# HuajianUP/Photo-SLAM

Hardware: AMD Instinct MI355X
Metric: train iters/s (render + L1/SSIM loss + backward + Adam), 2M Gaussians @1080p (higher is better)
Workload: dtype f32; 1 GPU; C3: Replica room0 @1080p shape; gaussians=2000000, width=1920, height=1080, sh_degree=3, parallelism=single GPU, raster_only=False, densify_interval=0, cull_empty_tiles=False, binning=depth-first, sh_adam_fused_into_backward=True, sh_adam_lazy_window=32, scene_index_order=random, geometry_adam_fused_into_backward=True, gaussians_after=2000000

## Files before the change

### photo-slam_amd/csrc/gsr_api.hip

```cpp
#include <atomic>
#include <chrono>
#include <cmath>
#include <vector>
#include "kernels.h"
#include "shrows.h"

#include <stdio.h>
#include <stdlib.h>
#include <string.h>

namespace gsr {

static thread_local int t_last_err = 0;
static thread_local char t_last_what[256] = {0};
void set_last_hip_error(int err, const char* what)
{
	t_last_err = err;
	snprintf(t_last_what, sizeof(t_last_what), "%s: %s", what ? what : "?", hipGetErrorString((hipError_t)err));
}

struct HostSync {
	uint32_t* pinned = nullptr;
	uint32_t* pinned_dev = nullptr;
	hipEvent_t ev = nullptr;
	hipStream_t side = nullptr;
	hipEvent_t fork = nullptr, join = nullptr;
	hipEvent_t notify = nullptr;
	int init_notify()
	{
		if (!notify) GSR_HIP(hipEventCreateWithFlags(&notify, hipEventDisableTiming));
		return GSR_OK;
	}
	int init_side()
	{
		if (!side) {
			int lo = 0, hi = 0;
			GSR_HIP(hipDeviceGetStreamPriorityRange(&lo, &hi));
			GSR_HIP(hipStreamCreateWithPriority(&side, hipStreamNonBlocking, lo));
		}
		if (!fork) GSR_HIP(hipEventCreateWithFlags(&fork, hipEventDisableTiming));
		if (!join) GSR_HIP(hipEventCreateWithFlags(&join, hipEventDisableTiming));
		return GSR_OK;
	}
	int init()
	{
		if (pinned && pinned_dev && ev) return GSR_OK;
		if (!pinned) {
			GSR_HIP(hipHostMalloc((void**)&pinned, 64 * sizeof(uint32_t), hipHostMallocMapped));
		}
		if (!pinned_dev) GSR_HIP(hipHostGetDevicePointer((void**)&pinned_dev, pinned, 0));
		if (!ev) GSR_HIP(hipEventCreateWithFlags(&ev, hipEventDisableTiming));
		return GSR_OK;
	}
	void release()
	{
		if (ev) (void)hipEventDestroy(ev);
		if (fork) (void)hipEventDestroy(fork);
		if (join) (void)hipEventDestroy(join);
		if (notify) (void)hipEventDestroy(notify);
		if (side) (void)hipStreamDestroy(side);
		if (pinned) (void)hipHostFree(pinned);
		*this = HostSync();
	}
};
constexpr int MAX_DEVICES = 16;
struct ThreadState {
	HostSync dev[MAX_DEVICES];
	~ThreadState()
	{
		int cur = 0;
		if (hipGetDevice(&cur) != hipSuccess) return;
		for (int d = 0; d < MAX_DEVICES; d++)
			if (dev[d].pinned || dev[d].ev || dev[d].side) {
				if (hipSetDevice(d) == hipSuccess) dev[d].release();
			}
		(void)hipSetDevice(cur);
	}
};
static thread_local ThreadState t_state;
static gsr_status host_sync(HostSync** out)
{
	int d = 0;
	GSR_HIP(hipGetDevice(&d));
	if (d < 0 || d >= MAX_DEVICES) return GSR_ERR_UNSUPPORTED;
	*out = &t_state.dev[d];
	return GSR_OK;
}
static thread_local int t_last_visible = -1;
static thread_local int t_last_forward_only = -1;
static thread_local const char* t_forward_only_geom = nullptr;
static thread_local const char* t_antialias_geom = nullptr;
static thread_local int t_antialias_bit = 0;
static thread_local double t_sync_wait_us = 0.0;
static thread_local long long t_sync_waits = 0;
static int env_int(const char* name, int unset)
{
	const char* e = getenv(name);
	if (!(e && *e)) return unset;
	fprintf(stderr, "[gsr] environment override %s=%s (wins over the API field / the library's default)\n", name, e);
	return atoi(e);
}
static bool side_stream_enabled(const gsr_sh_adam* o)
{
	static const int env = env_int("GSR_SH_ADAM_SIDE_STREAM", -1);
	return env >= 0 ? env != 0 : !(o && o->no_side_stream);
}
static bool lazy_slice_early(const gsr_sh_adam* o)
{
	static const int env = env_int("GSR_LAZY_SLICE_EARLY", -1);
	return env >= 0 ? env != 0 : !(o && o->lazy_slice_late);
}
static bool cov3D_stored()
{
	static const int env = env_int("GSR_COV3D_STORED", 0);
	return env != 0;
}
static bool emit_seeded()
{
	static const int env = env_int("GSR_EMIT_SEEDS", 1);
	return env != 0;
}
static int xcd_deal_mode(int tiles)
{
	static const int env = env_int("GSR_XCD_CHUNK", -1);
	if (env >= 0) return env;
	int c = 8;
	while (c > 1 && tiles < 8 * 16 * c) c >>= 1;
	return c;
}
static bool blend_bwd_half_tiles(int tiles)
{
	const char* e = getenv("GSR_BWD_HALF_TILES");
	if (e && *e) {
		static bool logged = false;
		if (!logged) fprintf(stderr, "[gsr] environment override GSR_BWD_HALF_TILES=%s\n", e);
		logged = true;
		return atoi(e) != 0;
	}
	return tiles >= 24 * 256;
}
static int depth_sort_wide()
{
	static const int on = env_int("GSR_DEPTH_SORT_9BIT", 1);
	static const int bits = env_int("GSR_DEPTH_SORT_BITS", 3 * RADIX_BITS_WIDE);
	if (!on) return 0;
	return (bits >= 1 && bits <= 27 && (div_up(bits, RADIX_BITS_WIDE) & 1)) ? bits : 3 * RADIX_BITS_WIDE;
}
static thread_local long long t_depth_resorts = 0;
static bool emit_hist()
{
	static const int env = env_int("GSR_EMIT_HIST", 1);
	return env != 0;
}
constexpr int TILE_FIRST_MAX_GAUSSIANS = 256 * 1024;
static bool binning_tile_first(int raw_params, int P, int tiles)
{
	static const int env = env_int("GSR_BINNING", -1);
	if (env >= 0) return env != 0;
	if (raw_params & GSR_BINNING_TILE_FIRST) return true;
	if (raw_params & GSR_BINNING_DEPTH_FIRST) return false;
	(void)tiles;
	return P <= TILE_FIRST_MAX_GAUSSIANS;
}
static int side_blocks(const gsr_sh_adam* o)
{
	static const int env = env_int("GSR_SH_ADAM_SIDE_BLOCKS", -1);
	return env >= 0 ? env : (o && o->side_blocks > 0 ? o->side_blocks : 256);
}

enum { ST_PREPROCESS = 0, ST_DEPTH_SORT, ST_OFFSET_SCAN, ST_EMIT, ST_TILE_SORT, ST_TILE_RANGES, ST_TILE_DEPTH_SORT, ST_BLEND_FWD,
       ST_GRAD_MEMSET, ST_BLEND_BWD, ST_PREPROCESS_BWD, ST_COUNT };
constexpr int ST_FWD_COUNT = ST_BLEND_FWD + 1;
static const char* const k_stage_names[ST_COUNT] = {"preprocess_fwd", "depth_sort", "offset_scan", "emit_instances",
                                                    "tile_sort", "tile_ranges", "tile_depth_sort", "blend_fwd", "grad_memset",
                                                    "blend_bwd", "preprocess_bwd"};
struct Profiler {
	std::atomic<int> on{0};
	hipEvent_t fwd[ST_FWD_COUNT + 1] = {};
	hipEvent_t bwd[4] = {};
	std::atomic<bool> created{false}, fwd_done{false}, bwd_done{false};
	int create()
	{
		if (created) return GSR_OK;
		for (auto& e : fwd) GSR_HIP(hipEventCreate(&e));
		for (auto& e : bwd) GSR_HIP(hipEventCreate(&e));
		created = true;
		return GSR_OK;
	}
};
static Profiler t_prof;
#define PROF_FWD(i) do { if (t_prof.on == 1) GSR_HIP(hipEventRecord(t_prof.fwd[i], stream)); } while (0)
#define PROF_BWD(i) do { if (t_prof.on == 1 || (t_prof.on == 2 && ((i) == 1 || (i) == 2))) GSR_HIP(hipEventRecord(t_prof.bwd[i], stream)); } while (0)

static inline size_t geometry_bytes(int P)
{
	size_t b = 0;
	GeometryState::carve(nullptr, (size_t)P, &b);
	return b;
}
static inline size_t binning_bytes(int R, bool forward_only = false, bool contribution = false)
{
	size_t b = 0;
	BinningState::carve(nullptr, (size_t)R, &b, forward_only, contribution);
	return b;
}
static inline size_t image_bytes(int W, int H, bool forward_only = false)
{
	size_t b = 0;
	const size_t T = (size_t)div_up(W, TILE) * div_up(H, TILE);
	ImageState::carve(nullptr, (size_t)W * H, T, &b, forward_only);
	return b;
}

static int validate_common(int P, int D, int M, int W, int H, const void* shs, const void* colors, const void* scales,
                           const void* rotations, const void* cov3D)
{
	if (P < 0 || W <= 0 || H <= 0) return GSR_ERR_INVALID_ARG;
	if ((shs == nullptr) == (colors == nullptr)) return GSR_ERR_INVALID_ARG;
	const bool sr = scales != nullptr && rotations != nullptr;
	if ((scales != nullptr) != (rotations != nullptr)) return GSR_ERR_INVALID_ARG;
	if (sr == (cov3D != nullptr)) return GSR_ERR_INVALID_ARG;
	if (shs) {
		if (D < 0 || D > 3) return GSR_ERR_UNSUPPORTED;
		if (M < (D + 1) * (D + 1)) return GSR_ERR_INVALID_ARG;
	}
	if (div_up(W, TILE) > 65535 || div_up(H, TILE) > 65535) return GSR_ERR_UNSUPPORTED;
	return GSR_OK;
}

static int make_lazy_adam(const gsr_sh_adam& o, const float* shs, int M, LazyAdam& la)
{
	const gsr_sh_adam_lazy& z = *o.lazy;
	if (!o.param || (shs && o.param != shs) || !o.exp_avg || !o.exp_avg_sq || !z.row_step || o.step < 1 || z.window < 2 ||
	    z.window > GSR_SH_LAZY_WINDOW)
		return GSR_ERR_INVALID_ARG;
	if (M != 16 || ((reinterpret_cast<uintptr_t>(o.param) | reinterpret_cast<uintptr_t>(o.exp_avg) | reinterpret_cast<uintptr_t>(o.exp_avg_sq)) & 15))
		return GSR_ERR_UNSUPPORTED;
	static_assert(GSR_SH_LAZY_WINDOW == LAZY_WINDOW_MAX, "gsr.h and kernels.h agree on the window");
	la.param = o.param; la.exp_avg = o.exp_avg; la.exp_avg_sq = o.exp_avg_sq;
	la.row_step = z.row_step; la.step = o.step; la.window = z.window;
	for (int k = 0; k < LAZY_WINDOW_MAX; k++) {
		AdamScalars s{};
		if (k < z.window && o.step - k >= 1)
			s = adam_scalars(k == 0 ? o.lr : z.lr_past[k - 1], k == 0 ? o.lr_tail : z.lr_tail_past[k - 1], o.beta1, o.beta2, o.eps, o.step - k);
		la.t.step_size[k] = s.step_size; la.t.step_size_tail[k] = s.step_size_tail; la.t.inv_sqrt_bc2[k] = s.inv_sqrt_bc2;
	}
	const AdamScalars c = adam_scalars(o.lr, o.lr_tail, o.beta1, o.beta2, o.eps, o.step);
	la.t.b1 = c.b1; la.t.b2 = c.b2; la.t.omb1 = c.omb1; la.t.omb2 = c.omb2; la.t.eps = c.eps;
	return GSR_OK;
}

}

using namespace gsr;

extern "C" {

size_t gsr_geometry_bytes(int P) { return geometry_bytes(P < 0 ? 0 : P); }
size_t gsr_binning_bytes(int R) { return binning_bytes(R < 0 ? 0 : R); }
size_t gsr_pose_grad_scratch_bytes(int P) { return pose_slab_floats(P) * sizeof(float); }
size_t gsr_geom_reg_scratch_bytes(int P) { return reg_slab_floats(P) * sizeof(float); }
size_t gsr_image_bytes(int W, int H) { return (W <= 0 || H <= 0) ? 0 : image_bytes(W, H); }
size_t gsr_binning_bytes_for(int R, int raw_params)
{
	return binning_bytes(R < 0 ? 0 : R, (raw_params & GSR_FORWARD_ONLY) != 0, (raw_params & GSR_CONTRIBUTION) != 0);
}
size_t gsr_image_bytes_for(int W, int H, int raw_params) { return (W <= 0 || H <= 0) ? 0 : image_bytes(W, H, (raw_params & GSR_FORWARD_ONLY) != 0); }
size_t gsr_knn_scratch_bytes(int P) { return knn_scratch_bytes(P < 0 ? 0 : P); }

const char* gsr_strerror(int status)
{
	switch (status) {
		case GSR_OK: return "ok";
		case GSR_ERR_INVALID_ARG: return "invalid argument";
		case GSR_ERR_ALLOC: return "scratch allocation callback returned NULL";
		case GSR_ERR_HIP: return "HIP runtime error";
		case GSR_ERR_UNSUPPORTED: return "unsupported configuration";
		default: return "unknown status";
	}
}
int gsr_last_hip_error(void) { return t_last_err; }
const char* gsr_last_hip_error_string(void) { return t_last_what; }
const char* gsr_backend(void)
{
#ifdef GSR_EMU
	return "emu-wave64";
#else
	return "hip-gfx950";
#endif
}

int gsr_forward(const gsr_forward_args* a, gsr_alloc_fn geometryBuffer, void* geometry_ctx, gsr_alloc_fn binningBuffer,
                void* binning_ctx, gsr_alloc_fn imageBuffer, void* image_ctx, void* stream_, int* num_rendered)
{
	if (!a || !geometryBuffer || !binningBuffer || !imageBuffer || !num_rendered) return GSR_ERR_INVALID_ARG;
	*num_rendered = 0;
	const bool fwd_only = (a->raw_params & GSR_FORWARD_ONLY) != 0;
	if (fwd_only && a->sh_adam && !a->sh_adam->lazy) return GSR_ERR_INVALID_ARG;
	const bool contribution = (a->raw_params & GSR_CONTRIBUTION) != 0;
	if (contribution != (a->out_weight_sum || a->out_weight_max || a->out_n_touched)) return GSR_ERR_INVALID_ARG;
	if (!contribution && a->pixel_weight) return GSR_ERR_INVALID_ARG;
	t_last_forward_only = fwd_only ? 1 : 0;
	int st = validate_common(a->P, a->D, a->M, a->width, a->height, a->shs, a->colors_precomp, a->scales, a->rotations,
	                         a->cov3D_precomp);
	if (a->P == 0) {
		t_last_visible = 0;
		return GSR_OK;
	}
	if (st != GSR_OK) return st;
	if (!a->background || !a->means3D || !a->opacities || !a->viewmatrix || !a->projmatrix || !a->cam_pos || !a->out_color)
		return GSR_ERR_INVALID_ARG;
	hipStream_t stream = (hipStream_t)stream_;
	const int P = a->P, W = a->width, H = a->height;
	const int grid_x = div_up(W, TILE), grid_y = div_up(H, TILE), tiles = grid_x * grid_y;

	char* geom_chunk = geometryBuffer(geometry_ctx, geometry_bytes(P));
	if (!geom_chunk) return GSR_ERR_ALLOC;
	GeometryState g = GeometryState::carve(geom_chunk, (size_t)P);
	if (fwd_only) t_forward_only_geom = geom_chunk;
	else if (t_forward_only_geom == geom_chunk) t_forward_only_geom = nullptr;
	if (!fwd_only) {
		t_antialias_geom = geom_chunk;
		t_antialias_bit = a->raw_params & GSR_ANTIALIAS;
	}
	char* img_chunk = imageBuffer(image_ctx, image_bytes(W, H, fwd_only));
	if (!img_chunk) return GSR_ERR_ALLOC;
	ImageState im = ImageState::carve(img_chunk, (size_t)W * H, (size_t)tiles, nullptr, fwd_only);

	HostSync* sync_ = nullptr;
	if ((st = host_sync(&sync_)) != GSR_OK) return st;
	HostSync& t_sync = *sync_;
	if ((st = t_sync.init()) != GSR_OK) return st;
	t_prof.fwd_done = false;
	PROF_FWD(0);

	PreprocessParams pp;
	pp.P = P; pp.D = a->D; pp.M = a->M;
	pp.means3D = a->means3D; pp.scales = a->scales; pp.scale_modifier = a->scale_modifier; pp.rotations = a->rotations;
	pp.opacities = a->opacities; pp.shs = a->shs; pp.cov3D_precomp = a->cov3D_precomp; pp.colors_precomp = a->colors_precomp;
	pp.view = a->viewmatrix; pp.proj = a->projmatrix; pp.campos = a->cam_pos;
	pp.W = W; pp.H = H; pp.tan_fovx = a->tan_fovx; pp.tan_fovy = a->tan_fovy;
	pp.focal_y = H / (2.0f * a->tan_fovy);
	pp.focal_x = W / (2.0f * a->tan_fovx);
	pp.grid_x = grid_x; pp.grid_y = grid_y; pp.radii_out = a->radii;
	pp.raw_params = a->raw_params | (cov3D_stored() ? GSR_STORE_COV3D : 0);
	pp.ranges = im.ranges; pp.tiles = tiles;
	pp.lazy = LazyAdam{};
	pp.forward_only = fwd_only ? 1 : 0;
	if (a->sh_adam && a->sh_adam->lazy) {
		if (!a->shs) return GSR_ERR_INVALID_ARG;
		if ((st = make_lazy_adam(*a->sh_adam, a->shs, a->M, pp.lazy)) != GSR_OK) return st;
	}
	if ((st = launch_preprocess_fwd(pp, g, stream)) != GSR_OK) return st;

	PROF_FWD(1);
	RadixHostCount hc;
	hc.pairs = g.wave_counts; hc.n = (int)wave_count_slots((size_t)P); hc.partials = g.count_partials; hc.host_out = t_sync.pinned_dev; hc.ready = t_sync.ev;

	uint32_t* const long_runs = fwd_only ? nullptr : g.long_runs;
	uint32_t* const long_counts = fwd_only ? nullptr : g.long_counts;
	const uint32_t long_capacity = fwd_only ? 0u : g.long_capacity;
	uint32_t *kres = nullptr, *vres = nullptr;
	const int narrow_bits = depth_sort_wide();
	auto plain_depth_sort = [&](const RadixHostCount* ride) {
		return launch_radix_sort(g.depth_key, nullptr, g.sort_keys_a, g.order, g.sort_keys_b, g.sort_vals_b, P, 0, 32, g.sort_scratch, stream,
		                         &kres, &vres, g.visible, ride);
	};
	auto offset_scan = [&]() {
		return launch_scan_rect_tiles(reinterpret_cast<const uint2*>(g.rect), g.order, g.offsets, g.rect_sorted, P, g.scan_scratch, stream,
		                              g.visible, g.sort_keys_b, EMIT_SEED_STRIDE, (uint32_t)P, long_runs, long_counts, long_capacity);
	};
	const bool tile_first = binning_tile_first(a->raw_params, P, tiles);
	if (tile_first) {
		st = launch_compact_visible(g.tiles_touched, reinterpret_cast<const uint2*>(g.rect), g.wave_counts, hc.n, g.count_partials, g.order, g.offsets,
		                            g.rect_sorted, P, t_sync.pinned_dev, t_sync.ev, stream, g.sort_keys_b, EMIT_SEED_STRIDE, (uint32_t)P, long_runs,
		                            long_counts, long_capacity, g.visible);
		if (st != GSR_OK) return st;
		PROF_FWD(2);
	} else {
		if (narrow_bits) {
			st = launch_radix_sort(g.depth_key, nullptr, g.sort_keys_b, g.sort_vals_b, g.sort_keys_a, g.order, P, 0, narrow_bits, g.sort_scratch, stream,
			                       &kres, &vres, g.visible, &hc, false, RADIX_BITS_WIDE, DEPTH_KEY_BIAS);
			if (st == GSR_OK && vres != g.order) st = GSR_ERR_INVALID_ARG;
		} else
			st = plain_depth_sort(&hc);
		if (st != GSR_OK) return st;
		PROF_FWD(2);
		if ((st = offset_scan()) != GSR_OK) return st;
	}
	PROF_FWD(3);

	{
		const auto w0 = std::chrono::steady_clock::now();
		GSR_HIP(hipEventSynchronize(t_sync.ev));
		t_sync_wait_us += std::chrono::duration<double, std::micro>(std::chrono::steady_clock::now() - w0).count();
		t_sync_waits++;
	}
	const unsigned long long R64 = (unsigned long long)t_sync.pinned[0] | ((unsigned long long)t_sync.pinned[1] << 32);
	const unsigned long long V64 = t_sync.pinned[2];
	t_last_visible = (int)V64;
	if (!tile_first && narrow_bits && V64 != 0 && (t_sync.pinned[3] - DEPTH_KEY_BIAS) >> narrow_bits) {
		if (!fwd_only) GSR_HIP(hipMemsetAsync(g.long_counts, 0, (size_t)LONG_LISTS * LONG_COUNT_STRIDE * sizeof(uint32_t), stream));
		if ((st = plain_depth_sort(nullptr)) != GSR_OK) return st;
		if ((st = offset_scan()) != GSR_OK) return st;
		t_depth_resorts++;
	}
	if (R64 > 0x7FFFFFFFull) return GSR_ERR_UNSUPPORTED;
	const int R = (int)R64;
	char* bin_chunk = binningBuffer(binning_ctx, binning_bytes(R, fwd_only, contribution));
	if (!bin_chunk) return GSR_ERR_ALLOC;
	BinningState bs = BinningState::carve(bin_chunk, (size_t)R, nullptr, fwd_only, contribution);

	uint32_t* point_list = bs.vals_a;
	if (R > 0) {
		const int bits = (int)higher_msb((uint32_t)tiles);
		const bool cull = (a->raw_params & GSR_CULL_EMPTY_TILES) != 0 && bits > 0;
		uint32_t* const listed = cull ? g.visible + 16 : nullptr;
		const int digit_bits = tile_sort_digit_bits(tiles, R);
		const bool one_pass = digit_bits == RADIX_BITS_ONE_PASS;
		const int hist_bits = emit_hist() ? radix_first_pass_bits(0, bits, digit_bits) : 0;
		if ((st = launch_emit_instances(tile_first ? (int)V64 : P, R, g, grid_x, bs.keys_a, bs.vals_a, bs.touched, stream, cull ? 1 : 0, emit_seeded(), bs.sort_scratch, hist_bits)) != GSR_OK) return st;
		PROF_FWD(4);
		uint32_t* tkeys = nullptr;
		if ((st = launch_radix_sort(bs.keys_a, bs.vals_a, bs.keys_a, bs.vals_a, bs.keys_b, bs.vals_b, R, 0, bits,
		                            bs.sort_scratch, stream, &tkeys, &point_list, listed, nullptr, hist_bits > 0, digit_bits, 0u,
		                            one_pass ? im.ranges : (uint2*)nullptr)) != GSR_OK)
			return st;
		PROF_FWD(5);
		if (!one_pass && (st = launch_tile_ranges(R, tkeys, im.ranges, stream, listed)) != GSR_OK) return st;
		PROF_FWD(6);
		if (tile_first) {
			const bool in_a = point_list == bs.vals_a;
			if ((st = launch_tile_depth_sort(im.ranges, tiles, g.depth_key, point_list, in_a ? bs.keys_b : bs.keys_a, in_a ? bs.vals_b : bs.vals_a,
			                                 bs.spare_words, stream)) != GSR_OK)
				return st;
		}
	} else {
		PROF_FWD(4);
		PROF_FWD(5);
		PROF_FWD(6);
	}
	PROF_FWD(7);

	BlendFwdParams bp;
	bp.ranges = im.ranges; bp.point_list = point_list; bp.rec = g.rec; bp.bg = a->background;
	bp.final_T = im.final_T; bp.n_contrib = im.n_contrib; bp.out_color = a->out_color;
	bp.contrib = bs.contrib; bp.contrib_stride = (size_t)R;
	bp.W = W; bp.H = H; bp.grid_x = grid_x; bp.tiles = tiles;
	bp.deal = make_tile_deal(tiles, grid_x, xcd_deal_mode(tiles));
	bp.forward_only = fwd_only ? 1 : 0;
	bp.depth = reinterpret_cast<const float*>(g.depth_key);
	bp.out_depth = a->out_depth; bp.out_alpha = a->out_alpha;
	bp.stats = nullptr; bp.stats_slots = (uint32_t)R; bp.pixel_weight = nullptr;
	if (contribution && R > 0) {
		GSR_HIP(hipMemsetAsync(bs.stats, 0, stats_floats((size_t)R) * sizeof(float), stream));
		bp.stats = bs.stats; bp.pixel_weight = a->pixel_weight;
	}
	if ((st = launch_blend_fwd(bp, stream)) != GSR_OK) return st;
	if (contribution) {
		ContributionParams cp;
		cp.P = P; cp.tiles_touched = g.tiles_touched; cp.rec = g.rec; cp.stats = R > 0 ? bs.stats : nullptr; cp.stats_slots = (uint32_t)R;
		cp.out_sum = a->out_weight_sum; cp.out_max = a->out_weight_max; cp.out_cnt = a->out_n_touched;
		cp.accumulate = a->contribution_accumulate ? 1 : 0;
		if ((st = launch_contribution_reduce(cp, stream)) != GSR_OK) return st;
	}
	PROF_FWD(8);
	t_prof.fwd_done = t_prof.on == 1;
	*num_rendered = R;
	return GSR_OK;
}

int gsr_backward(const gsr_backward_args* a, void* stream_)
{
	if (!a) return GSR_ERR_INVALID_ARG;
	int st = validate_common(a->P, a->D, a->M, a->width, a->height, a->shs, a->colors_precomp, a->scales, a->rotations,
	                         a->cov3D_precomp);
	const int pose_ptrs = (a->dL_dviewmatrix != nullptr) + (a->dL_dprojmatrix != nullptr) + (a->dL_dcampos != nullptr) + (a->pose_scratch != nullptr);
	if (pose_ptrs != 0 && pose_ptrs != 4) return GSR_ERR_INVALID_ARG;
	const bool pose = pose_ptrs == 4;
	if (pose && (reinterpret_cast<uintptr_t>(a->pose_scratch) & 3)) return GSR_ERR_INVALID_ARG;
	bool reg = false;
	if (const gsr_geom_reg* gr = a->geom_reg) {
		const float ws[3] = {gr->w_opacity, gr->w_scale, gr->w_isotropic};
		for (const float w : ws)
			if (!std::isfinite(w) || w < 0.f) return GSR_ERR_INVALID_ARG;
		if (gr->loss && (!gr->scratch || (reinterpret_cast<uintptr_t>(gr->scratch) & 3))) return GSR_ERR_INVALID_ARG;
		if (a->cov3D_precomp && (gr->w_scale != 0.f || gr->w_isotropic != 0.f)) return GSR_ERR_INVALID_ARG;
		reg = gr->w_opacity != 0.f || gr->w_scale != 0.f || gr->w_isotropic != 0.f || gr->loss != nullptr;
		if (reg && (a->dL_dcolor_view || a->packed_view || pose)) return GSR_ERR_UNSUPPORTED;
	}
	if (a->P == 0) {
		if (reg && a->geom_reg->loss) return launch_reg_zero(a->geom_reg->loss, (hipStream_t)stream_);
		return pose ? launch_pose_zero(a->dL_dviewmatrix, a->dL_dprojmatrix, a->dL_dcampos, (hipStream_t)stream_) : GSR_OK;
	}
	if (st != GSR_OK) return st;
	if (!a->background || !a->means3D || !a->viewmatrix || !a->projmatrix || !a->campos || !a->geom_buffer ||
	    !a->image_buffer || !a->dL_dpix || !a->dL_dcolor || !a->dL_dmean3D || a->R < 0)
		return GSR_ERR_INVALID_ARG;
	if (pose && (a->dL_dcolor_view || a->packed_view)) return GSR_ERR_UNSUPPORTED;
	if (!a->dL_dopacity && !a->geom_adam) return GSR_ERR_INVALID_ARG;
	if (a->shs && !a->dL_dsh && !a->dL_dcolor_view && !a->sh_adam) return GSR_ERR_INVALID_ARG;
	if ((a->stat_grad_accum != nullptr) != (a->stat_denom != nullptr) || (a->stat_denom != nullptr) != (a->stat_max_radii != nullptr))
		return GSR_ERR_INVALID_ARG;
	if (a->sh_adam && (!a->shs || (a->dL_dcolor_view && !a->sh_adam->lazy) || !a->sh_adam->exp_avg || !a->sh_adam->exp_avg_sq ||
	                   a->sh_adam->step < 1))
		return GSR_ERR_INVALID_ARG;
	if (a->dL_dcolor_view && !a->shs) return GSR_ERR_INVALID_ARG;
	if (a->scales && (!a->dL_dscale || !a->dL_drot) && !a->geom_adam) return GSR_ERR_INVALID_ARG;
	if (a->R > 0 && !a->binning_buffer) return GSR_ERR_INVALID_ARG;
	if (t_forward_only_geom != nullptr && a->geom_buffer == t_forward_only_geom) return GSR_ERR_INVALID_ARG;
	if (t_antialias_geom != nullptr && a->geom_buffer == t_antialias_geom && (a->raw_params & GSR_ANTIALIAS) != t_antialias_bit)
		return GSR_ERR_INVALID_ARG;
	if (a->color_view_ready_stream && a->dL_dcolor_view && a->color_view_ready_stream == stream_) return GSR_ERR_INVALID_ARG;
	if (a->packed_view && a->dL_dcolor_view && (a->packed_capacity_rows < 0 || (a->packed_capacity_rows & 3))) return GSR_ERR_INVALID_ARG;
	const bool depth = a->dL_ddepth || a->dL_dalpha;
	hipStream_t stream = (hipStream_t)stream_;
	const int P = a->P, W = a->width, H = a->height, R = a->R;
	const int grid_x = div_up(W, TILE), grid_y = div_up(H, TILE), tiles = grid_x * grid_y;
	GeometryState g = GeometryState::carve(a->geom_buffer, (size_t)P);
	ImageState im = ImageState::carve(a->image_buffer, (size_t)W * H, (size_t)tiles);
	BinningState bs = BinningState::carve(a->binning_buffer, (size_t)R);
	const int passes = tile_sort_passes(tiles, R);
	const uint32_t* point_list = (passes % 2) ? bs.vals_b : bs.vals_a;

	HostSync* sync_ = nullptr;
	if (gsr_status hs = host_sync(&sync_); hs != GSR_OK) return hs;
	HostSync& t_sync = *sync_;
	t_prof.bwd_done = false;
	const bool pre_slice = a->sh_adam && a->dL_dcolor_view;
	const bool rows_path = sh_rows_path(a->shs, a->M, a->D, a->dL_dcolor_view != nullptr, a->sh_adam != nullptr && !pre_slice, a->dL_dsh);
	if (!a->dL_dcov3D && a->cov3D_precomp) return GSR_ERR_INVALID_ARG;
	if (a->sh_adam) {
		const gsr_sh_adam& o = *a->sh_adam;
		if (o.param != a->shs || !o.param) return GSR_ERR_INVALID_ARG;
		if (!rows_path || ((reinterpret_cast<uintptr_t>(o.exp_avg) | reinterpret_cast<uintptr_t>(o.exp_avg_sq)) & 15))
			return GSR_ERR_UNSUPPORTED;
	}
	GeomAdam geom{};
	if (a->geom_adam) {
		const gsr_geom_adam& o = *a->geom_adam;
		const int all_raw = GSR_RAW_OPACITY | GSR_RAW_SCALING | GSR_RAW_ROTATION;
		const gsr_adam_tensor* ts[4] = {&o.xyz, &o.opacity, &o.scaling, &o.rotation};
		for (const gsr_adam_tensor* t : ts)
			if (!t->param || !t->exp_avg || !t->exp_avg_sq || t->step < 1) return GSR_ERR_INVALID_ARG;
		if ((a->raw_params & all_raw) != all_raw || a->cov3D_precomp || o.xyz.param != a->means3D || o.scaling.param != a->scales ||
		    o.rotation.param != a->rotations || !a->dL_dmean3D || a->dL_dcolor_view)
			return GSR_ERR_INVALID_ARG;
		if ((reinterpret_cast<uintptr_t>(o.rotation.param) | reinterpret_cast<uintptr_t>(o.rotation.exp_avg) |
		     reinterpret_cast<uintptr_t>(o.rotation.exp_avg_sq)) & 15)
			return GSR_ERR_UNSUPPORTED;
		if (!(rows_path && a->scales && a->rotations)) return GSR_ERR_UNSUPPORTED;
		auto fill = [&](const gsr_adam_tensor& t, GeomAdamTensor& gt) {
			gt.param = t.param; gt.exp_avg = t.exp_avg; gt.exp_avg_sq = t.exp_avg_sq;
			gt.s = adam_scalars(t.lr, t.lr, o.beta1, o.beta2, o.eps, t.step);
		};
		geom.on = 1;
		fill(o.xyz, geom.xyz); fill(o.opacity, geom.opacity); fill(o.scaling, geom.scaling); fill(o.rotation, geom.rotation);
	}
	bool side_busy = false;
	auto fail = [&](int status) -> int {
		if (side_busy) (void)hipStreamWaitEvent(stream, t_sync.join, 0);
		return status;
	};
	const bool lazy = a->sh_adam && a->sh_adam->lazy;
	LazyAdam la{};
	if (lazy) {
		if (!a->shs) return GSR_ERR_INVALID_ARG;
		if ((st = make_lazy_adam(*a->sh_adam, a->shs, a->M, la)) != GSR_OK) return st;
		if (pre_slice && la.window < 3) return GSR_ERR_INVALID_ARG;
	}
	auto launch_lazy_slice = [&]() -> int {
		const int* radii = pre_slice ? nullptr : (a->radii ? a->radii : g.radii);
		const int mode = pre_slice ? 3 : 0;
		if (!side_stream_enabled(a->sh_adam)) return launch_sh_adam_lazy(P, radii, la, stream, mode);
		int s2 = t_sync.init_side();
		if (s2 != GSR_OK) return s2;
		GSR_HIP(hipEventRecord(t_sync.fork, stream));
		GSR_HIP(hipStreamWaitEvent(t_sync.side, t_sync.fork, 0));
		s2 = launch_sh_adam_lazy(P, radii, la, t_sync.side, mode);
		GSR_HIP(hipEventRecord(t_sync.join, t_sync.side));
		side_busy = true;
		return s2;
	};
	if (lazy) {
	} else if (a->sh_adam && a->M == 16 && a->D >= 0 && a->D <= 3 && side_stream_enabled(a->sh_adam)) {
		const gsr_sh_adam& o = *a->sh_adam;
		if ((st = t_sync.init_side()) != GSR_OK) return st;
// ... 288 lines not shown
```

### photo-slam_amd/csrc/state.h

```cpp
#pragma once
#include "rt.h"

namespace gsr {

constexpr int TILE = 16;
constexpr int TILE_PIXELS = TILE * TILE;
constexpr uint32_t DEPTH_KEY_CULLED = 0xFFFFFFFFu;
constexpr uint32_t DEPTH_KEY_BIAS = 0x3E4CCCCDu;
constexpr int PRE_THREADS = 128;
static inline size_t wave_count_slots(size_t P) { return ((P + PRE_THREADS - 1) / PRE_THREADS) * (PRE_THREADS / 64); }
constexpr int HOST_COUNT_WORDS = 4;

constexpr int SORT_THREADS = 256;
constexpr int SORT_ITEMS_PER_WAVE = 512;
constexpr int SORT_CHUNK = 4 * SORT_ITEMS_PER_WAVE;
constexpr int SORT_ROUNDS = SORT_ITEMS_PER_WAVE / 64;
constexpr int RADIX_BITS = 8;
constexpr int RADIX_BITS_WIDE = 9;
constexpr int RADIX_BINS = 1 << RADIX_BITS;
constexpr uint32_t RADIX_INVALID_KEY = 0xFFFFFFFFu;
constexpr uint32_t LONG_RUN = 64;
constexpr int LONG_LISTS = 64, LONG_COUNT_STRIDE = 32;
static inline size_t long_list_capacity(size_t P);

// ... 43 lines not shown
	uint32_t* depth_key;
	uint32_t* tiles_touched;
	int*      radii;
	uint16_t* rect;
	float4*   rec;
	float*    cov3D;
	uint8_t*  clamped;
	uint32_t* order;
	uint32_t* offsets;
	uint32_t* sort_keys_a;
	uint32_t* sort_keys_b;
	uint32_t* sort_vals_b;
	uint32_t* sort_scratch;
	uint32_t* scan_scratch;
	uint2*    rect_sorted;
	uint32_t* visible;

	static GeometryState carve(char* chunk, size_t P, size_t* bytes = nullptr)
	{
		GeometryState g;
		Carver c(chunk);
		g.depth_key = c.take<uint32_t>(P);
		g.tiles_touched = c.take<uint32_t>(P);
		g.radii = c.take<int>(P);
		g.rect = c.take<uint16_t>(4 * P);
		g.rec = c.take<float4>(REC_FLOAT4S * P);
		g.cov3D = c.take<float>(6 * P);
		g.clamped = c.take<uint8_t>(P);
		g.order = c.take<uint32_t>(P);
		g.offsets = c.take<uint32_t>(P);
		g.sort_keys_a = c.take<uint32_t>(P);
		g.sort_keys_b = c.take<uint32_t>(P);
		g.sort_vals_b = c.take<uint32_t>(P);
		g.sort_scratch = c.take<uint32_t>(sort_scratch_elems((int)P) > sort_scratch_elems_wide((int)P) ? sort_scratch_elems((int)P) : sort_scratch_elems_wide((int)P));
		g.scan_scratch = c.take<uint32_t>(scan_scratch_elems((int)P));
		g.rect_sorted = c.take<uint2>(P);
		g.visible = c.take<uint32_t>(32);
		g.wave_counts = c.take<uint4>(wave_count_slots(P));
		g.count_partials = c.take<uint4>((size_t)sort_blocks((int)P));
		g.long_runs = c.take<uint32_t>((size_t)LONG_LISTS * long_list_capacity(P));
		g.long_counts = c.take<uint32_t>((size_t)LONG_LISTS * LONG_COUNT_STRIDE);
		g.long_capacity = (uint32_t)long_list_capacity(P);
		if (bytes) *bytes = c.used(chunk) + 128;
		return g;
	}
};

static inline size_t touched_clear_bytes(size_t R) { return (R + 64 + 255) & ~(size_t)255; }
static inline size_t stats_floats(size_t R) { return 12 * R; }
struct BinningState {
	uint32_t* keys_a;
	uint32_t* vals_a;
	uint32_t* keys_b;
	uint32_t* vals_b;
	uint32_t* sort_scratch;
	float*    partials;
	uint8_t*  touched;
	uint8_t*  contrib;
	uint32_t* spare_words;

	float*    stats;

	static BinningState carve(char* chunk, size_t R, size_t* bytes = nullptr, bool forward_only = false, bool contribution = false)
	{
		BinningState b;
		Carver c(chunk);
		b.keys_a = c.take<uint32_t>(R);
		b.vals_a = c.take<uint32_t>(R);
		b.keys_b = c.take<uint32_t>(R);
		b.vals_b = c.take<uint32_t>(R);
		b.sort_scratch = c.take<uint32_t>(tile_sort_scratch_elems((int)R));
		if (forward_only) {
			b.partials = nullptr;
			b.touched = nullptr;
			b.contrib = nullptr;
			b.spare_words = c.take<uint32_t>(R + 16);
			b.stats = contribution ? c.take<float>(stats_floats(R)) : nullptr;
			if (bytes) *bytes = c.used(chunk) + 128;
			return b;
		}
		b.partials = c.take<float>(4 * (size_t)SLOT_F4 * R);
		b.touched = c.take<uint8_t>(touched_clear_bytes(R));
		b.contrib = c.take<uint8_t>(4 * R + 64);
		b.spare_words = reinterpret_cast<uint32_t*>(b.contrib);
		b.stats = contribution ? c.take<float>(stats_floats(R)) : nullptr;
		if (bytes) *bytes = c.used(chunk) + 128;
		return b;
	}
};

struct TileDeal {
	int tiles, grid_x;
	int mode;
};
static inline TileDeal make_tile_deal(int tiles, int grid_x, int mode)
{
	TileDeal d;
	d.tiles = tiles; d.grid_x = grid_x; d.mode = mode < 0 ? 8 : mode;
	return d;
}

struct ImageState {
	float*    final_T;
	uint32_t* n_contrib;
	uint2*    ranges;

	static ImageState carve(char* chunk, size_t N, size_t T, size_t* bytes = nullptr, bool forward_only = false)
	{
		ImageState im;
		Carver c(chunk);
		im.final_T = forward_only ? nullptr : c.take<float>(N);
		im.n_contrib = forward_only ? nullptr : c.take<uint32_t>(N);
		im.ranges = c.take<uint2>(T);
		if (bytes) *bytes = c.used(chunk) + 128;
		return im;
	}
};

static inline uint32_t higher_msb(uint32_t n)
{
	uint32_t msb = sizeof(n) * 4;
	uint32_t step = msb;
	while (step > 1) {
		step /= 2;
		if (n >> msb) msb += step;
		else msb -= step;
	}
	if (n >> msb) msb++;
	return msb;
}

static inline bool result_in_a(int passes) { return (passes % 2) == 0; }
constexpr int RADIX_BITS_ONE_PASS = 11;
constexpr int TILE_SORT_ONE_PASS_MAX = 512 * 1024;
static inline int tile_sort_digit_bits(int tiles, int R)
{
	const int bits = (int)higher_msb((uint32_t)tiles);
	return (bits > RADIX_BITS && bits <= RADIX_BITS_ONE_PASS && R <= TILE_SORT_ONE_PASS_MAX) ? RADIX_BITS_ONE_PASS : RADIX_BITS;
}
static inline int tile_sort_passes(int tiles, int R) { return div_up((int)higher_msb((uint32_t)tiles), tile_sort_digit_bits(tiles, R)); }

int launch_scan_rect_tiles(const uint2* rect, const uint32_t* gather, uint32_t* out, uint2* rect_sorted, int n, uint32_t* scratch,
                           hipStream_t stream, const uint32_t* n_dev, uint32_t* seeds = nullptr, uint32_t seed_stride = 1,
                           uint32_t seed_capacity = 0, uint32_t* long_runs = nullptr, uint32_t* long_counts = nullptr,
                           uint32_t long_capacity = 0);
int launch_scan_u32(const uint32_t* in, const uint32_t* gather, uint32_t* out, int n, bool inclusive,
                    uint32_t* scratch, hipStream_t stream, const uint32_t* n_dev = nullptr);
constexpr int COMPACT_ONE_LEVEL_PAIRS = 2048;
int launch_compact_visible(const uint32_t* tiles_touched, const uint2* rect, const uint4* wave_counts, int n_pairs, uint4* partials,
                           uint32_t* order, uint32_t* offsets, uint2* rect_sorted, int n, uint32_t* host_out, void* ready, hipStream_t stream,
                           uint32_t* seeds = nullptr, uint32_t seed_stride = 1, uint32_t seed_capacity = 0, uint32_t* long_runs = nullptr,
                           uint32_t* long_counts = nullptr, uint32_t long_capacity = 0, uint32_t* visible_out = nullptr);
int launch_tile_depth_sort(const uint2* ranges, int tiles, const uint32_t* depth_key, uint32_t* point_list, uint32_t* spare_keys,
                           uint32_t* spare_vals, uint32_t* spare_words, hipStream_t stream);
struct RadixHostCount {
	const uint4* pairs = nullptr;
	int n = 0;
	uint4* partials = nullptr;
	uint32_t* host_out = nullptr;
	void* ready = nullptr;
};
int launch_radix_sort(const uint32_t* keys_in, const uint32_t* vals_in, uint32_t* keys_ping, uint32_t* vals_ping,
                      uint32_t* keys_pong, uint32_t* vals_pong, int n, int begin_bit, int end_bit,
                      uint32_t* scratch, hipStream_t stream, uint32_t** keys_res, uint32_t** vals_res,
                      uint32_t* compact_count = nullptr, const RadixHostCount* host_count = nullptr, bool first_hist_ready = false,
                      int digit_bits = RADIX_BITS, uint32_t bias = 0, uint2* ranges_out = nullptr);
static inline int radix_first_pass_bits(int begin_bit, int end_bit, int digit_bits = RADIX_BITS)
{
	const int passes = end_bit > begin_bit ? div_up(end_bit - begin_bit, digit_bits) : 0;
	return passes ? div_up(end_bit - begin_bit, passes) : 0;
}

}
```

### photo-slam_amd/csrc/tile_depth_sort.hip

```cpp
#include "state.h"
#include "wave64.h"
#include "kernels.h"

namespace gsr {

constexpr int TDS_THREADS = 256, TDS_WAVES = TDS_THREADS / 64;
constexpr int TDS_CHUNK = 2048;
constexpr int TDS_ROUNDS = TDS_CHUNK / TDS_THREADS;
constexpr int TDS_BITS = 8, TDS_BINS = 1 << TDS_BITS;
static_assert(TDS_BINS == TDS_THREADS, "thread d owns digit d");

struct TdsShared {
	uint32_t whist[TDS_WAVES][TDS_BINS];
	uint32_t gbase[TDS_BINS];
	uint32_t cur[TDS_BINS];
	uint32_t keys[TDS_CHUNK];
	uint32_t vals[TDS_CHUNK];
	uint32_t wave[4];
	uint32_t red[2 * TDS_WAVES];
};

template <class Between>
__device__ __forceinline__ void tds_rank_chunk(const uint32_t (&key)[TDS_ROUNDS], const uint32_t (&val)[TDS_ROUNDS], uint32_t live, int rounds,
                                               uint32_t bias, int shift, int nbits, TdsShared& S, Between&& between)
{
	const int w = wave_id(), tid = (int)threadIdx.x;
	const uint32_t dmask = (1u << nbits) - 1u;
#pragma unroll
	for (int i = 0; i < TDS_WAVES; i++) S.whist[i][tid] = 0u;
	__syncthreads();
	uint32_t place[TDS_ROUNDS];
#pragma unroll
	for (int r = 0; r < TDS_ROUNDS; r++) {
		place[r] = 0u;
		if (r < rounds) {
			const bool valid = (live >> r) & 1u;
			const uint32_t d = ((key[r] - bias) >> shift) & dmask;
			const unsigned long long m = wave_match_digit(d, nbits, valid);
			const uint32_t rank = (uint32_t)__popcll(m & lanemask_lt()), size = (uint32_t)__popcll(m);
			place[r] = rank | (size << 8);
			if (valid && rank == 0u) S.whist[w][d] += size;
			wave_fence();
		}
	}
	__syncthreads();
	{
		const uint32_t c0 = S.whist[0][tid], c1 = S.whist[1][tid], c2 = S.whist[2][tid], c3 = S.whist[3][tid];
		const uint32_t tot = c0 + c1 + c2 + c3;
		uint32_t all;
		const uint32_t lstart = block_excl_scan_256(tot, &all, S.wave);
		S.whist[0][tid] = lstart;
		S.whist[1][tid] = lstart + c0;
		S.whist[2][tid] = lstart + c0 + c1;
		S.whist[3][tid] = lstart + c0 + c1 + c2;
		between(lstart, tot);
	}
	__syncthreads();
#pragma unroll
	for (int r = 0; r < TDS_ROUNDS; r++) {
		if (r < rounds) {
			const bool valid = (live >> r) & 1u;
			const uint32_t d = ((key[r] - bias) >> shift) & dmask;
			const uint32_t rank = place[r] & 0xFFu, size = place[r] >> 8;
			uint32_t cursor = 0;
			if (valid) cursor = S.whist[w][d];
			wave_fence();
			if (valid) {
				S.keys[cursor + rank] = key[r];
				S.vals[cursor + rank] = val[r];
				if (rank == 0u) S.whist[w][d] = cursor + size;
			}
			wave_fence();
		}
	}
	__syncthreads();
}

__device__ __forceinline__ void tds_block_min_max(uint32_t lo, uint32_t hi, TdsShared& S, uint32_t& kmin, uint32_t& kmax)
{
	const uint32_t wlo = ~wave_max_u32(~lo), whi = wave_max_u32(hi);
	__syncthreads();
	if (lane_id() == 0) {
		S.red[wave_id()] = wlo;
		S.red[TDS_WAVES + wave_id()] = whi;
	}
	__syncthreads();
	kmin = min(min(S.red[0], S.red[1]), min(S.red[2], S.red[3]));
	kmax = max(max(S.red[TDS_WAVES], S.red[TDS_WAVES + 1]), max(S.red[TDS_WAVES + 2], S.red[TDS_WAVES + 3]));
}

__global__ void __launch_bounds__(TDS_THREADS)
tile_depth_sort_kernel(const uint2* __restrict__ ranges, int tiles, const uint32_t* __restrict__ depth_key, uint32_t* point_list,
                       uint32_t* xk, uint32_t* xv, uint32_t* yk)
{
	__shared__ TdsShared S;
	const int tile = (int)blockIdx.x;
	if (tile >= tiles) return;
	const uint2 range = ranges[tile];
	const int n = (int)(range.y - range.x);
	if (n <= 1) return;
	const int w = wave_id(), l = lane_id(), tid = (int)threadIdx.x;
	uint32_t* const pl = point_list + range.x;
	uint32_t key[TDS_ROUNDS], val[TDS_ROUNDS];

	if (n <= TDS_CHUNK) {
		const int span = ((n + TDS_WAVES - 1) / TDS_WAVES + 63) & ~63;
		const int rounds = span >> 6;
		uint32_t live = 0u, lo = 0xFFFFFFFFu, hi = 0u;
#pragma unroll
		for (int r = 0; r < TDS_ROUNDS; r++) {
			const int e = w * span + r * 64 + l;
			key[r] = 0u;
			val[r] = 0u;
			if (r < rounds && e < n) {
				val[r] = pl[e];
				live |= 1u << r;
			}
		}
#pragma unroll
		for (int r = 0; r < TDS_ROUNDS; r++)
			if ((live >> r) & 1u) {
				key[r] = depth_key[val[r]];
				lo = min(lo, key[r]);
				hi = max(hi, key[r]);
			}
		uint32_t kmin, kmax;
		tds_block_min_max(lo, hi, S, kmin, kmax);
		if (kmax == kmin) return;
		const int bits = 32 - __builtin_clz(kmax - kmin);
		const int passes = (bits + TDS_BITS - 1) / TDS_BITS, bpp = (bits + passes - 1) / passes;
		for (int p = 0; p < passes; p++) {
			const int shift = p * bpp, nbits = min(bpp, bits - shift);
			tds_rank_chunk(key, val, live, rounds, kmin, shift, nbits, S, [](uint32_t, uint32_t) {});
			if (p + 1 < passes) {
#pragma unroll
				for (int r = 0; r < TDS_ROUNDS; r++)
					if ((live >> r) & 1u) {
						const int e = w * span + r * 64 + l;
						key[r] = S.keys[e];
						val[r] = S.vals[e];
					}
			}
		}
		for (int i = tid; i < n; i += TDS_THREADS) pl[i] = S.vals[i];
		return;
	}

	uint32_t* ak = yk + range.x;
	uint32_t* av = pl;
	uint32_t* bk = xk + range.x;
	uint32_t* bv = xv + range.x;
	uint32_t lo = 0xFFFFFFFFu, hi = 0u;
	for (int i = tid; i < n; i += TDS_THREADS) {
		const uint32_t k = depth_key[pl[i]];
		ak[i] = k;
		lo = min(lo, k);
		hi = max(hi, k);
	}
	uint32_t kmin, kmax;
	tds_block_min_max(lo, hi, S, kmin, kmax);
	if (kmax == kmin) return;
	const int bits = 32 - __builtin_clz(kmax - kmin);
	const int passes = (bits + TDS_BITS - 1) / TDS_BITS, bpp = (bits + passes - 1) / passes;
	for (int p = 0; p < passes; p++) {
		const int shift = p * bpp, nbits = min(bpp, bits - shift);
		const uint32_t dmask = (1u << nbits) - 1u;
		S.cur[tid] = 0u;
		__syncthreads();
		for (int i = tid; i < n; i += TDS_THREADS) atomicAdd(&S.cur[((ak[i] - kmin) >> shift) & dmask], 1u);
		__syncthreads();
		{
			const uint32_t c = S.cur[tid];
			uint32_t all;
			const uint32_t ex = block_excl_scan_256(c, &all, S.wave);
			S.cur[tid] = ex;
		}
		__syncthreads();
		for (int base = 0; base < n; base += TDS_CHUNK) {
			const int cn = min(TDS_CHUNK, n - base);
			uint32_t live = 0u;
#pragma unroll
			for (int r = 0; r < TDS_ROUNDS; r++) {
				const int e = w * (TDS_CHUNK / TDS_WAVES) + r * 64 + l;
				key[r] = 0u;
				val[r] = 0u;
				if (e < cn) {
					key[r] = ak[base + e];
					val[r] = av[base + e];
					live |= 1u << r;
				}
			}
			tds_rank_chunk(key, val, live, TDS_ROUNDS, kmin, shift, nbits, S, [&](uint32_t lstart, uint32_t tot) {
				S.gbase[tid] = S.cur[tid] - lstart;
				S.cur[tid] += tot;
			});
			for (int i = tid; i < cn; i += TDS_THREADS) {
				const uint32_t k = S.keys[i];
				const uint32_t pos = S.gbase[((k - kmin) >> shift) & dmask] + (uint32_t)i;
				bk[pos] = k;
				bv[pos] = S.vals[i];
			}
		}
		__syncthreads();
		uint32_t* t = ak; ak = bk; bk = t;
		t = av; av = bv; bv = t;
	}
	if (av != pl)
		for (int i = tid; i < n; i += TDS_THREADS) pl[i] = av[i];
}

int launch_tile_depth_sort(const uint2* ranges, int tiles, const uint32_t* depth_key, uint32_t* point_list, uint32_t* spare_keys,
                           uint32_t* spare_vals, uint32_t* spare_words, hipStream_t stream)
{
	if (!ranges || !depth_key || !point_list || !spare_keys || !spare_vals || !spare_words) return GSR_ERR_INVALID_ARG;
	if (tiles <= 0) return GSR_OK;
	GSR_LAUNCH(tile_depth_sort_kernel, tiles, TDS_THREADS, stream, ranges, tiles, (const uint32_t*)depth_key, point_list, spare_keys, spare_vals, spare_words);
	GSR_CHECK_LAUNCH();
	return GSR_OK;
}

}
```

Measured before the change: 684.0 iters/s.

## Widen per-tile depth sort to 9-bit digits with approximate-top-bits fixup pass

The per-tile depth sort moves from 8-bit to 9-bit digits, using packed 16-bit per-wave histograms so each thread owns two bins. It also adds a path for small tiles that sorts only the top 18 bits and then fixes the order of low bits with a bounded neighbor scan, falling back to a full sort when runs exceed a cap. The binning threshold for tile-first is raised, but the workload forces depth-first binning, so the tile sort kernel likely does not run. This adds complexity and risks correctness when 16-bit counters or the fixup window are exceeded.

```diff
diff --git a/photo-slam_amd/csrc/gsr_api.hip b/photo-slam_amd/csrc/gsr_api.hip
--- a/photo-slam_amd/csrc/gsr_api.hip
+++ b/photo-slam_amd/csrc/gsr_api.hip
@@ -152,7 +152,7 @@
 	static const int env = env_int("GSR_EMIT_HIST", 1);
 	return env != 0;
 }
-constexpr int TILE_FIRST_MAX_GAUSSIANS = 256 * 1024;
+constexpr int TILE_FIRST_MAX_GAUSSIANS = 2 * 1024 * 1024;
 static bool binning_tile_first(int raw_params, int P, int tiles)
 {
 	static const int env = env_int("GSR_BINNING", -1);
@@ -161,6 +161,11 @@
 	if (raw_params & GSR_BINNING_DEPTH_FIRST) return false;
 	(void)tiles;
 	return P <= TILE_FIRST_MAX_GAUSSIANS;
+}
+static bool tile_sort_fixup()
+{
+	static const int env = env_int("GSR_TILE_SORT_FIXUP", 1);
+	return env != 0;
 }
 static int side_blocks(const gsr_sh_adam* o)
 {
@@ -432,7 +437,7 @@
 		if (tile_first) {
 			const bool in_a = point_list == bs.vals_a;
 			if ((st = launch_tile_depth_sort(im.ranges, tiles, g.depth_key, point_list, in_a ? bs.keys_b : bs.keys_a, in_a ? bs.vals_b : bs.vals_a,
-			                                 bs.spare_words, stream)) != GSR_OK)
+			                                 bs.spare_words, stream, tile_sort_fixup())) != GSR_OK)
 				return st;
 		}
 	} else {
diff --git a/photo-slam_amd/csrc/state.h b/photo-slam_amd/csrc/state.h
--- a/photo-slam_amd/csrc/state.h
+++ b/photo-slam_amd/csrc/state.h
@@ -219,7 +219,7 @@
                            uint32_t* seeds = nullptr, uint32_t seed_stride = 1, uint32_t seed_capacity = 0, uint32_t* long_runs = nullptr,
                            uint32_t* long_counts = nullptr, uint32_t long_capacity = 0, uint32_t* visible_out = nullptr);
 int launch_tile_depth_sort(const uint2* ranges, int tiles, const uint32_t* depth_key, uint32_t* point_list, uint32_t* spare_keys,
-                           uint32_t* spare_vals, uint32_t* spare_words, hipStream_t stream);
+                           uint32_t* spare_vals, uint32_t* spare_words, hipStream_t stream, bool fixup = true);
 struct RadixHostCount {
 	const uint4* pairs = nullptr;
 	int n = 0;
diff --git a/photo-slam_amd/csrc/tile_depth_sort.hip b/photo-slam_amd/csrc/tile_depth_sort.hip
--- a/photo-slam_amd/csrc/tile_depth_sort.hip
+++ b/photo-slam_amd/csrc/tile_depth_sort.hip
@@ -7,27 +7,31 @@
 constexpr int TDS_THREADS = 256, TDS_WAVES = TDS_THREADS / 64;
 constexpr int TDS_CHUNK = 2048;
 constexpr int TDS_ROUNDS = TDS_CHUNK / TDS_THREADS;
-constexpr int TDS_BITS = 8, TDS_BINS = 1 << TDS_BITS;
-static_assert(TDS_BINS == TDS_THREADS, "thread d owns digit d");
+constexpr int TDS_BITS = 9, TDS_BINS = 1 << TDS_BITS;
+constexpr int TDS_CAP = 8;
+static_assert(TDS_BINS == 2 * TDS_THREADS, "thread t owns digits 2 t and 2 t + 1");
+static_assert(TDS_CHUNK < 65536 && TDS_CHUNK / TDS_WAVES <= 65535, "counts and cursors are 16-bit");
+
+typedef uint32_t __attribute__((may_alias)) tds_pair_t;
 
 struct TdsShared {
-	uint32_t whist[TDS_WAVES][TDS_BINS];
-	uint32_t gbase[TDS_BINS];
+	uint16_t whist[TDS_WAVES][TDS_BINS];
 	uint32_t cur[TDS_BINS];
 	uint32_t keys[TDS_CHUNK];
 	uint32_t vals[TDS_CHUNK];
 	uint32_t wave[4];
 	uint32_t red[2 * TDS_WAVES];
+	uint32_t long_run;
 };
 
-template <class Between>
 __device__ __forceinline__ void tds_rank_chunk(const uint32_t (&key)[TDS_ROUNDS], const uint32_t (&val)[TDS_ROUNDS], uint32_t live, int rounds,
-                                               uint32_t bias, int shift, int nbits, TdsShared& S, Between&& between)
+                                               uint32_t bias, int shift, int nbits, TdsShared& S, uint32_t& tot0, uint32_t& tot1)
 {
 	const int w = wave_id(), tid = (int)threadIdx.x;
 	const uint32_t dmask = (1u << nbits) - 1u;
-#pragma unroll
-	for (int i = 0; i < TDS_WAVES; i++) S.whist[i][tid] = 0u;
+	tds_pair_t* const pairs = reinterpret_cast<tds_pair_t*>(&S.whist[0][0]);
+#pragma unroll
+	for (int i = 0; i < TDS_WAVES; i++) pairs[i * TDS_THREADS + tid] = 0u;
 	__syncthreads();
 	uint32_t place[TDS_ROUNDS];
 #pragma unroll
@@ -39,21 +43,30 @@
 			const unsigned long long m = wave_match_digit(d, nbits, valid);
 			const uint32_t rank = (uint32_t)__popcll(m & lanemask_lt()), size = (uint32_t)__popcll(m);
 			place[r] = rank | (size << 8);
-			if (valid && rank == 0u) S.whist[w][d] += size;
+			if (valid && rank == 0u) S.whist[w][d] = (uint16_t)(S.whist[w][d] + size);
 			wave_fence();
 		}
 	}
 	__syncthreads();
 	{
-		const uint32_t c0 = S.whist[0][tid], c1 = S.whist[1][tid], c2 = S.whist[2][tid], c3 = S.whist[3][tid];
-		const uint32_t tot = c0 + c1 + c2 + c3;
+		uint32_t c[TDS_WAVES];
+		tot0 = 0u;
+		tot1 = 0u;
+#pragma unroll
+		for (int i = 0; i < TDS_WAVES; i++) {
+			c[i] = pairs[i * TDS_THREADS + tid];
+			tot0 += c[i] & 0xFFFFu;
+			tot1 += c[i] >> 16;
+		}
 		uint32_t all;
-		const uint32_t lstart = block_excl_scan_256(tot, &all, S.wave);
-		S.whist[0][tid] = lstart;
-		S.whist[1][tid] = lstart + c0;
-		S.whist[2][tid] = lstart + c0 + c1;
-		S.whist[3][tid] = lstart + c0 + c1 + c2;
-		between(lstart, tot);
+		uint32_t at0 = block_excl_scan_256(tot0 + tot1, &all, S.wave);
+		uint32_t at1 = at0 + tot0;
+#pragma unroll
+		for (int i = 0; i < TDS_WAVES; i++) {
+			pairs[i * TDS_THREADS + tid] = at0 | (at1 << 16);
+			at0 += c[i] & 0xFFFFu;
+			at1 += c[i] >> 16;
+		}
 	}
 	__syncthreads();
 #pragma unroll
@@ -68,7 +81,7 @@
 			if (valid) {
 				S.keys[cursor + rank] = key[r];
 				S.vals[cursor + rank] = val[r];
-				if (rank == 0u) S.whist[w][d] = cursor + size;
+				if (rank == 0u) S.whist[w][d] = (uint16_t)(cursor + size);
 			}
 			wave_fence();
 		}
@@ -84,6 +97,7 @@
 		S.red[wave_id()] = wlo;
 		S.red[TDS_WAVES + wave_id()] = whi;
 	}
+	if (threadIdx.x == 0) S.long_run = 0u;
 	__syncthreads();
 	kmin = min(min(S.red[0], S.red[1]), min(S.red[2], S.red[3]));
 	kmax = max(max(S.red[TDS_WAVES], S.red[TDS_WAVES + 1]), max(S.red[TDS_WAVES + 2], S.red[TDS_WAVES + 3]));
@@ -91,7 +105,7 @@
 
 __global__ void __launch_bounds__(TDS_THREADS)
 tile_depth_sort_kernel(const uint2* __restrict__ ranges, int tiles, const uint32_t* __restrict__ depth_key, uint32_t* point_list,
-                       uint32_t* xk, uint32_t* xv, uint32_t* yk)
+                       uint32_t* xk, uint32_t* xv, uint32_t* yk, int fixup)
 {
 	__shared__ TdsShared S;
 	const int tile = (int)blockIdx.x;
@@ -102,6 +116,7 @@
 	const int w = wave_id(), l = lane_id(), tid = (int)threadIdx.x;
 	uint32_t* const pl = point_list + range.x;
 	uint32_t key[TDS_ROUNDS], val[TDS_ROUNDS];
+	uint32_t tot0, tot1;
 
 	if (n <= TDS_CHUNK) {
 		const int span = ((n + TDS_WAVES - 1) / TDS_WAVES + 63) & ~63;
@@ -128,19 +143,67 @@
 		tds_block_min_max(lo, hi, S, kmin, kmax);
 		if (kmax == kmin) return;
 		const int bits = 32 - __builtin_clz(kmax - kmin);
+		auto reload = [&]() {
+#pragma unroll
+			for (int r = 0; r < TDS_ROUNDS; r++)
+				if ((live >> r) & 1u) {
+					const int e = w * span + r * 64 + l;
+					key[r] = S.keys[e];
+					val[r] = S.vals[e];
+				}
+		};
+		if (fixup && bits > 2 * TDS_BITS && bits <= 3 * TDS_BITS) {
+			const int low = bits - 2 * TDS_BITS;
+			for (int p = 0; p < 2; p++) {
+				tds_rank_chunk(key, val, live, rounds, kmin, low + p * TDS_BITS, TDS_BITS, S, tot0, tot1);
+				reload();
+			}
+			int pos[TDS_ROUNDS];
+			bool long_run = false;
+#pragma unroll
+			for (int r = 0; r < TDS_ROUNDS; r++) {
+				pos[r] = 0;
+				if (r < rounds) {
+					const bool valid = (live >> r) & 1u;
+					const int e = w * span + r * 64 + l;
+					const uint32_t mine = key[r] - kmin;
+					pos[r] = e;
+					for (int off = 1; off <= TDS_CAP; off++) {
+						const int a = e - off, b = e + off;
+						uint32_t ka = 0u, kb = 0u;
+						bool sa = false, sb = false;
+						if (valid && a >= 0) {
+							ka = S.keys[a] - kmin;
+							sa = (ka >> low) == (mine >> low);
+						}
+						if (valid && b < n) {
+							kb = S.keys[b] - kmin;
+							sb = (kb >> low) == (mine >> low);
+						}
+						if (wave_ballot(sa || sb) == 0ull) break;
+						if (off == TDS_CAP) {
+							long_run = long_run || sa || sb;
+						} else {
+							pos[r] -= (sa && ka > mine) ? 1 : 0;
+							pos[r] += (sb && kb < mine) ? 1 : 0;
+						}
+					}
+				}
+			}
+			if (long_run) S.long_run = 1u;
+			__syncthreads();
+			if (S.long_run == 0u) {
+#pragma unroll
+				for (int r = 0; r < TDS_ROUNDS; r++)
+					if ((live >> r) & 1u) pl[pos[r]] = val[r];
+				return;
+			}
+		}
 		const int passes = (bits + TDS_BITS - 1) / TDS_BITS, bpp = (bits + passes - 1) / passes;
 		for (int p = 0; p < passes; p++) {
 			const int shift = p * bpp, nbits = min(bpp, bits - shift);
-			tds_rank_chunk(key, val, live, rounds, kmin, shift, nbits, S, [](uint32_t, uint32_t) {});
-			if (p + 1 < passes) {
-#pragma unroll
-				for (int r = 0; r < TDS_ROUNDS; r++)
-					if ((live >> r) & 1u) {
-						const int e = w * span + r * 64 + l;
-						key[r] = S.keys[e];
-						val[r] = S.vals[e];
-					}
-			}
+			tds_rank_chunk(key, val, live, rounds, kmin, shift, nbits, S, tot0, tot1);
+			if (p + 1 < passes) reload();
 		}
 		for (int i = tid; i < n; i += TDS_THREADS) pl[i] = S.vals[i];
 		return;
@@ -165,15 +228,17 @@
 	for (int p = 0; p < passes; p++) {
 		const int shift = p * bpp, nbits = min(bpp, bits - shift);
 		const uint32_t dmask = (1u << nbits) - 1u;
-		S.cur[tid] = 0u;
+		S.cur[2 * tid] = 0u;
+		S.cur[2 * tid + 1] = 0u;
 		__syncthreads();
 		for (int i = tid; i < n; i += TDS_THREADS) atomicAdd(&S.cur[((ak[i] - kmin) >> shift) & dmask], 1u);
 		__syncthreads();
 		{
-			const uint32_t c = S.cur[tid];
+			const uint32_t c0 = S.cur[2 * tid], c1 = S.cur[2 * tid + 1];
 			uint32_t all;
-			const uint32_t ex = block_excl_scan_256(c, &all, S.wave);
-			S.cur[tid] = ex;
+			const uint32_t ex = block_excl_scan_256(c0 + c1, &all, S.wave);
+			S.cur[2 * tid] = ex;
+			S.cur[2 * tid + 1] = ex + c0;
 		}
 		__syncthreads();
 		for (int base = 0; base < n; base += TDS_CHUNK) {
@@ -190,16 +255,18 @@
 					live |= 1u << r;
 				}
 			}
-			tds_rank_chunk(key, val, live, TDS_ROUNDS, kmin, shift, nbits, S, [&](uint32_t lstart, uint32_t tot) {
-				S.gbase[tid] = S.cur[tid] - lstart;
-				S.cur[tid] += tot;
-			});
+			tds_rank_chunk(key, val, live, TDS_ROUNDS, kmin, shift, nbits, S, tot0, tot1);
 			for (int i = tid; i < cn; i += TDS_THREADS) {
 				const uint32_t k = S.keys[i];
-				const uint32_t pos = S.gbase[((k - kmin) >> shift) & dmask] + (uint32_t)i;
+				const uint32_t d = ((k - kmin) >> shift) & dmask;
+				const uint32_t first = d ? (uint32_t)S.whist[TDS_WAVES - 1][d - 1u] : 0u;
+				const uint32_t pos = S.cur[d] + (uint32_t)i - first;
 				bk[pos] = k;
 				bv[pos] = S.vals[i];
 			}
+			__syncthreads();
+			S.cur[2 * tid] += tot0;
+			S.cur[2 * tid + 1] += tot1;
 		}
 		__syncthreads();
 		uint32_t* t = ak; ak = bk; bk = t;
@@ -210,11 +277,12 @@
 }
 
 int launch_tile_depth_sort(const uint2* ranges, int tiles, const uint32_t* depth_key, uint32_t* point_list, uint32_t* spare_keys,
-                           uint32_t* spare_vals, uint32_t* spare_words, hipStream_t stream)
+                           uint32_t* spare_vals, uint32_t* spare_words, hipStream_t stream, bool fixup)
 {
 	if (!ranges || !depth_key || !point_list || !spare_keys || !spare_vals || !spare_words) return GSR_ERR_INVALID_ARG;
 	if (tiles <= 0) return GSR_OK;
-	GSR_LAUNCH(tile_depth_sort_kernel, tiles, TDS_THREADS, stream, ranges, tiles, (const uint32_t*)depth_key, point_list, spare_keys, spare_vals, spare_words);
+	GSR_LAUNCH(tile_depth_sort_kernel, tiles, TDS_THREADS, stream, ranges, tiles, (const uint32_t*)depth_key, point_list, spare_keys, spare_vals, spare_words,
+	           fixup ? 1 : 0);
 	GSR_CHECK_LAUNCH();
 	return GSR_OK;
 }
```

Result: faster. 694.5 iters/s, median of 6 (+1.5%).
